# dpbriggs/Distributed-Sieve-e

Measured on AMD Instinct MI355X. Metric: sieved integers/sec at N=1e11, 1/2/4/8 MI355X; % of LDS/HBM roofline, higher is better.
Workload: dtype u32; 1 GPU; N=1e+11 odd-only chunked sieve, P=1 spread-work chunks (one per GPU), mask resident in HBM; N=100000000000, P=1, cs=49999999999, mask_bytes_per_gpu=6250000000, parallelism=range-partition x1 (RCCL broadcast + all-reduce)

## Files before the change

### distributed-sieve-e_amd/csrc/dse_host.cpp

```cpp
#include <rccl/rccl.h>

#include <algorithm>
#include <cmath>
#include <cstdio>
#include <cstring>
#include <string>
#include <vector>

#include "../../include/dse.h"
#include "dse_internal.h"

namespace {

thread_local std::string g_err;
thread_local int32_t g_code = DSE_OK;

int32_t fail(int32_t code, const std::string& msg) {
  g_err = msg;
  g_code = code;
  return code;
}

#define HIP_TRY(expr)                                                                     \
  do {                                                                                    \
    hipError_t e_ = (expr);                                                               \
    if (e_ != hipSuccess)                                                                 \
      return fail(DSE_EHIP, std::string(#expr " failed: ") + hipGetErrorString(e_));      \
  } while (0)

#define NCCL_TRY(expr)                                                                    \
  do {                                                                                    \
    ncclResult_t r_ = (expr);                                                             \
    if (r_ != ncclSuccess)                                                                \
      return fail(DSE_ENCCL, std::string(#expr " failed: ") + ncclGetErrorString(r_));    \
  } while (0)

uint64_t isqrt_u64(uint64_t x) {
  uint64_t r = (uint64_t)std::sqrt((long double)x);
  while (r > 0 && r * r > x) --r;
  while ((r + 1) * (r + 1) <= x) ++r;
  return r;
}

uint32_t prime_cap(uint64_t x) {
  if (x < 100) return 64;
  double b = 1.25506 * (double)x / std::log((double)x);
  return (uint32_t)b + 64;
}

struct ChunkMask {
  int32_t my_num = 0;
  uint64_t* dev_ptr = nullptr;
  uint64_t words = 0;
};

struct DevState {
  int device = 0;
  int num_cus = 0;
  hipStream_t stream = nullptr;
  void* table = nullptr;
  uint64_t table_bytes = 0;
  unsigned long long* counts = nullptr;
// ... 623 lines not shown
      return fail(DSE_EINVAL, "rccl_single needs a one-device context (dse_init(1) or dse_init_device)");
    if (value == 1 && ctx->comms.empty()) {
      int dev = ctx->devs[0].device;
      HIP_TRY(hipSetDevice(dev));
      ncclComm_t c;
      NCCL_TRY(ncclCommInitAll(&c, 1, &dev));
      ctx->comms.push_back(c);
    } else if (value == 0 && !ctx->comms.empty()) {
      HIP_TRY(hipSetDevice(ctx->devs[0].device));
      HIP_TRY(hipStreamSynchronize(ctx->devs[0].stream));
      NCCL_TRY(ncclCommDestroy(ctx->comms[0]));
      ctx->comms.clear();
    }
    ctx->rccl_single = value == 1;
    return DSE_OK;
  }
  if (n == "table_broadcast_max_bytes") {
    if (value < 0) return fail(DSE_EINVAL, "table_broadcast_max_bytes must be >= 0");
    ctx->opts.table_bcast_max = (uint64_t)value;
    return DSE_OK;
  }
  if (n == "bucket_cap_divisor") {
    if (value < 0 || value > 0xFFFFFFFFll) return fail(DSE_EINVAL, "bucket_cap_divisor out of range");
    ctx->opts.bucket_cap_div = (uint32_t)value;
    return DSE_OK;
  }
  return fail(DSE_EINVAL, "unknown option " + n);
}

int32_t dse_debug_get_stat(dse_ctx* ctx, const char* name, int64_t* value) {
  if (!ctx || !name || !value) return fail(DSE_EINVAL, "null ctx, stat name or value");
  const std::string n(name);
  if (n == "rccl_calls") {
    *value = ctx->rccl_calls;
    return DSE_OK;
  }
  if (n == "table_local_builds") {
    *value = ctx->table_local_builds;
    return DSE_OK;
  }
  if (n == "rccl_comms") {
    *value = (int64_t)ctx->comms.size();
    return DSE_OK;
  }
  if (n == "rccl_ranks") {
    int c = 0;
    if (!ctx->comms.empty()) NCCL_TRY(ncclCommCount(ctx->comms[0], &c));
    *value = c;
    return DSE_OK;
  }
  return fail(DSE_EINVAL, "unknown stat " + n);
}

}

namespace {

inline int fmt_u64(uint64_t v, char* out) {
  char t[24];
  int n = 0;
  do {
    t[n++] = (char)('0' + v % 10);
    v /= 10;
  } while (v);
  for (int i = 0; i < n; ++i) out[i] = t[n - 1 - i];
  return n;
}

inline int fmt_java_double(uint64_t v, char* out) {
  if (v < 10000000ull) {
    int n = fmt_u64(v, out);
    out[n++] = '.';
    out[n++] = '0';
    return n;
  }
  char d[24];
  int len = fmt_u64(v, d);
  int sig = len;
  while (sig > 1 && d[sig - 1] == '0') --sig;
  int n = 0;
  out[n++] = d[0];
  out[n++] = '.';
  if (sig == 1) out[n++] = '0';
  for (int i = 1; i < sig; ++i) out[n++] = d[i];
  out[n++] = 'E';
  n += fmt_u64((uint64_t)(len - 1), out + n);
  return n;
}

}

extern "C" int32_t dse_write_range_file(const char* path, int32_t my_num, uint64_t g_start, uint64_t nbits,
                                        const uint64_t* mask) {
  if (!path || !mask) return fail(DSE_EINVAL, "null path or mask");
  if (my_num < 1) return fail(DSE_EINVAL, "my_num must be >= 1");
  if (my_num == 1 && nbits < 4) return fail(DSE_EINVAL, "finish's 2/3/5/7 hack needs a chunk of >= 4 candidates");
  const uint64_t cs = nbits;
  FILE* f = std::fopen(path, "wb");
  if (!f) return fail(DSE_EIO, std::string("cannot open ") + path);
  std::vector<char> buf(1 << 20);
  size_t used = 0;
  int per_line = 0;
  const uint64_t base = g_start;
  auto emit = [&](uint64_t v) {
    if (used + 64 > buf.size()) {
      std::fwrite(buf.data(), 1, used, f);
// ... 47 lines not shown
```

### distributed-sieve-e_amd/csrc/dse_wheel_args.h

```cpp
#pragma once
#include <algorithm>
#include <vector>

#include "dse_wheel_geometry.h"

namespace dse {
namespace {

WheelRange make_wheel_range(const RangeSpec& rs, uint64_t* plane_lut) {
  WheelRange w{};
  const uint64_t v_start = 3 + 2 * rs.g_start;
  w.V0 = v_start - 1;
  w.nbits = rs.nbits;
  w.KB0 = w.V0 / 30;
  w.out = rs.out;
  w.count = rs.count;
  const uint32_t v0m = (uint32_t)(w.V0 % 30);
  uint32_t n = 0;
  *plane_lut = 0;
  for (uint32_t rho = 1; rho < 30; rho += 2) {
    const uint32_t r = (v0m + rho) % 30;
    if (r % 3 == 0 || r % 5 == 0) continue;
    uint32_t iota = 0;
    while (kR30[iota] != r) ++iota;
    w.rho_pack |= (uint64_t)rho << (5 * n);
    w.pl_pack |= n << (3 * iota);
    if (v0m + rho >= 30) w.e_iota |= 1u << iota;
    *plane_lut |= (uint64_t)n << (3 * (rho >> 1));
    ++n;
  }
  constexpr uint32_t small[] = {3, 5, 7, 11, 13, 17, 19, 23, 29, 31, 37, 41, 43, 47, 53, 59, 61, 67, 71, 73, 79};
  static_assert(small[sizeof(small) / sizeof(small[0]) - 1] == kQMax && (kQMax - 3) / 2 < 64, "fix covers 3..kQMax");
  for (uint32_t v : small)
    if (v >= v_start && (v - v_start) / 2 < rs.nbits) w.fix |= 1ull << ((v - v_start) / 2);
  for (int g = 0; g < kNG; ++g) w.v0g[g] = (uint16_t)(w.V0 % gmod(g));
  return w;
}

uint64_t isqrt64(uint64_t x) {
  uint64_t r = (uint64_t)__builtin_sqrt((double)x);
  while (r * r > x) --r;
  while ((r + 1) * (r + 1) <= x) ++r;
  return r;
}

WheelArgs make_wheel_args(const RangeSpec* rs, uint32_t n, uint64_t* plane_lut,
                          uint64_t wheel_max = kWheelMaxPrime) {
  static const std::vector<uint32_t> odd_primes = [] {
    std::vector<uint8_t> comp(kWheelMaxPrime / 2 + 1, 0);
    for (uint64_t i = 1; (2 * i + 1) * (2 * i + 1) <= kWheelMaxPrime; ++i)
      if (!comp[i])
        for (uint64_t j = ((2 * i + 1) * (2 * i + 1)) / 2; j <= kWheelMaxPrime / 2; j += 2 * i + 1) comp[j] = 1;
    std::vector<uint32_t> v;
    for (uint64_t i = 1; 2 * i + 1 <= kWheelMaxPrime; ++i)
      if (!comp[i]) v.push_back((uint32_t)(2 * i + 1));
    return v;
  }();
  const uint64_t lim[5] = {kQMax, TA, TB1, TB, std::min<uint64_t>(wheel_max, kWheelMaxPrime)};
  WheelArgs wa{};
  for (int t = 0; t < 5; ++t)
    wa.nthr[t] = (uint32_t)(std::upper_bound(odd_primes.begin(), odd_primes.end(), lim[t]) - odd_primes.begin());
  uint64_t seg = 0, lut = 0;
  for (uint32_t i = 0; i < n; ++i) {
    WheelRange& r = wa.r[i];
    r = make_wheel_range(rs[i], i ? &lut : plane_lut);
    r.seg0 = (uint32_t)seg;
    const uint64_t nseg_r = (rs[i].nbits + kWheelOutBits - 1) / kWheelOutBits;
    seg += nseg_r;
    r.lsh = 0;
    while (nseg_r > 0 && ((nseg_r - 1) >> r.lsh) >= kLPieces) ++r.lsh;
// ... 28 lines not shown
```

### distributed-sieve-e_amd/csrc/dse_wheel_geometry.h

```cpp
#pragma once
#include <hip/hip_runtime.h>
#include <stddef.h>
#include <stdint.h>

#include <algorithm>

#include "dse_internal.h"

namespace dse {
namespace {

constexpr uint32_t KP = 1u << kWheelLogKP;
constexpr uint32_t BLOCKS = KP / 32;
constexpr uint32_t IMG_WORDS = 8 * BLOCKS;
constexpr uint32_t IMG_BYTES = 4 * IMG_WORDS;
static_assert(IMG_BYTES == KP, "a period index is its block's byte address");
#define DSE_IMG_OFF_S "32768"
constexpr uint32_t kImgOff = 32768;
#define DSE_STR2(x) #x
#define DSE_STR(x) DSE_STR2(x)
constexpr uint32_t NT = 1024;
constexpr uint32_t NW = NT / 64;
static_assert(BLOCKS % (64 * NW) == 0, "expansion blocks");
#ifndef DSE_TA
// ... 26 lines not shown
constexpr uint32_t gmod(int g) { return kGQ[g][0] * kGQ[g][1] * kGQ[g][2]; }
constexpr uint32_t kInitWords = IMG_WORDS / NT;
constexpr uint32_t kInitRun = 32 * kInitWords;
constexpr uint32_t kExpandBlocks = BLOCKS / NW;
constexpr uint32_t kInitBlocks = kInitRun / 128 + 2;
constexpr uint32_t gdw(int g) { return ((gmod(g) + 32 * (4 * kInitBlocks + 1) + 127) / 128) * 4; }
constexpr uint32_t gbase(int g) { return g == 0 ? 0u : gbase(g - 1) + gdw(g - 1); }
constexpr uint32_t kGDW = gbase(kNG);
constexpr uint32_t kGInv30[kNG] = {inv30_const(gmod(0)), inv30_const(gmod(1)), inv30_const(gmod(2)),
                                   inv30_const(gmod(3)), inv30_const(gmod(4)), inv30_const(gmod(5)),
                                   inv30_const(gmod(6)), inv30_const(gmod(7)), inv30_const(gmod(8))};

struct InitTables {
  uint32_t w[4 * kGDW];
};
constexpr InitTables make_init_tables() {
  InitTables t{};
  for (int g = 0; g < kNG; ++g) {
    for (uint32_t j = 0; j < gdw(g) + 3; ++j) {
      uint32_t v = 0;
      for (uint32_t b = 0; b < 32; ++b) {
        const uint32_t y = 32 * j + b;
        const bool hit = y % kGQ[g][0] == 0 || y % kGQ[g][1] == 0 || (kGQ[g][2] > 1 && y % kGQ[g][2] == 0);
        v |= (uint32_t)hit << b;
      }
      for (uint32_t k = 0; k < 4; ++k)
        if (j >= k && j - k < gdw(g)) t.w[k * kGDW + gbase(g) + (j - k)] = v;
    }
  }
  return t;
}
__device__ const InitTables g_init_tables = make_init_tables();

constexpr uint32_t kLPieces = 16;
constexpr uint32_t kMaxRanges = 9;

}


struct WheelRange {
  uint64_t V0;
  uint64_t nbits;
  uint64_t KB0;
  uint64_t rho_pack;
  uint32_t* out;
  unsigned long long* count;
  uint32_t pl_pack;
  uint32_t e_iota;
  uint64_t fix;
  uint32_t seg0;
  uint16_t v0g[kNG];
  uint32_t lsh;
  uint32_t lcap[kLPieces];
};

struct WheelArgs {
  WheelRange r[kMaxRanges];
  uint32_t nranges;
  uint32_t nseg;
  uint32_t nthr[5];
  const uint32_t* bk_entries;
  const uint32_t* bk_start;
  const uint32_t* bk_reg0;
  const uint32_t* bk_n0;
  const unsigned long long* bk_spill;
  const uint32_t* bk_nspill;
  uint64_t bk_spill_cap;
  uint32_t bk_k0;
};
static_assert(sizeof(WheelArgs) <= 4096, "kernel arguments");
static_assert(alignof(WheelArgs) <= 8, "kernel argument layout");

namespace {

constexpr uint32_t kWaOffset = 8;

#ifndef DSE_BK_GRID
#define DSE_BK_GRID 1024
#endif
#ifndef DSE_BK_UNIT_BATCHES
#define DSE_BK_UNIT_BATCHES 4
#endif
constexpr uint32_t kBkBatchU = 16;
constexpr uint32_t kBkUnit = 64 * kBkBatchU * DSE_BK_UNIT_BATCHES;
constexpr uint32_t kBkGrid0 = DSE_BK_GRID;
#ifndef DSE_BK0_LISTS
#define DSE_BK0_LISTS 16
#endif
constexpr uint32_t kBk0Lists = DSE_BK0_LISTS;
static_assert(kBkGrid0 % kBk0Lists == 0 && 64 % kBk0Lists == 0, "band-0 bucket units");
constexpr uint32_t kKeyShift = 20;
static_assert(IMG_WORDS * 32 <= (1u << kKeyShift), "bucket entry layout");

}
}
```

### distributed-sieve-e_amd/csrc/dse_wheel_kernel.h

```cpp
#pragma once
#include "dse_wheel_geometry.h"

namespace dse {
namespace {

__device__ __forceinline__ uint32_t lds_addr(const uint32_t* p) {
  return (uint32_t)(uintptr_t)(const __attribute__((address_space(3))) uint32_t*)p;
}

__device__ __forceinline__ void lds_drain() { asm volatile("s_waitcnt lgkmcnt(0)" ::: "memory"); }

__device__ __forceinline__ uint32_t opaque(uint32_t x) {
  asm volatile("" : "+v"(x));
  return x;
}

constexpr uint32_t kBlockMask = ~31u;
#ifndef DSE_FAKE_CF_L
#define DSE_FAKE_CF_L 0
#endif
constexpr uint32_t kBlockMaskL = DSE_FAKE_CF_L ? ~127u : kBlockMask;
#ifndef DSE_FAKE_CF_INIT
#define DSE_FAKE_CF_INIT 0
#endif
#ifndef DSE_SHORT_TAIL
#define DSE_SHORT_TAIL 16
#endif
constexpr uint32_t kShortTail = DSE_SHORT_TAIL;
constexpr uint32_t odd_primes_upto(uint32_t x) {
  uint32_t c = 0;
  for (uint32_t v = 3; v <= x; v += 2) {
    bool pr = true;
    for (uint32_t d = 3; d * d <= v; d += 2)
      if (v % d == 0) { pr = false; break; }
    c += pr;
  }
  return c;
}
constexpr uint32_t kL0 = odd_primes_upto(TB);
constexpr uint32_t kLPrimeMask = 0x800FFFFFu;
static_assert(kWheelMaxPrime <= (1u << 20), "pl[] words: the L primes (odd, <= kWheelMaxPrime) are below 2^20");
__host__ __device__ constexpr uint32_t l_plan(uint32_t pmin, uint32_t pmax, uint32_t kp) {
  if (pmin > kp) return 2;
  if (pmin > kp / 2) return 1;
  const uint32_t n_min = pmax >= kp ? 0u : kp / pmax;
  const uint32_t n_all = (kp + pmin - 1) / pmin;
  return n_all - n_min <= kShortTail ? n_all << 3 : 4u | n_min << 3;
}
static_assert(l_plan(TB + 2, TB + 2, 1u << 17) < (1u << 11) && l_plan(TB + 2, TB + 2, 1u << 16) < (1u << 11),
              "the plan fits bits 20..30 of a pl[] word (bit 31: kLPrimeMask's dead-lane flag)");
static_assert(odd_primes_upto(kQMax) + kMidCap >= kL0, "the L list starts at kL0 whenever it exists");

__device__ __forceinline__ void mark_k(uint32_t pb4, uint32_t k, uint32_t one) {
// ... 126 lines not shown
  return (uint32_t)r;
}

__device__ __forceinline__ float fast_rcp(float x) { return __builtin_amdgcn_rcpf(x); }

__device__ __forceinline__ uint32_t div_ceil_small(uint32_t t, uint32_t p, float invp) {
  uint32_t q = (uint32_t)((float)t * invp);
  q = q * p > t ? q - 1 : q;
  q = (q + 1) * p <= t ? q + 1 : q;
  return q + (q * p != t ? 1u : 0u);
}

__device__ __forceinline__ uint32_t div_small(uint32_t t, uint32_t p, float invp) {
  uint32_t q = (uint32_t)((float)t * invp);
  q = q * p > t ? q - 1 : q;
  q = (q + 1) * p <= t ? q + 1 : q;
  return q;
}

__device__ __forceinline__ uint32_t mulmod_small(uint32_t x, uint32_t y, uint32_t p, float invp) {
  const uint32_t xy = x * y;
  uint32_t q = (uint32_t)((float)xy * invp);
  int32_t r = (int32_t)(xy - q * p);
  r = r < 0 ? r + (int32_t)p : r;
  r = r < 0 ? r + (int32_t)p : r;
  r = r >= (int32_t)p ? r - (int32_t)p : r;
  r = r >= (int32_t)p ? r - (int32_t)p : r;
  return (uint32_t)r;
}

__host__ __device__ __forceinline__ uint64_t inv30_of(uint64_t p) {
  constexpr uint64_t T = (14ull << 0) | (8ull << 12) | (9ull << 20) | (11ull << 24) | (3ull << 32) | (5ull << 36) |
                         (6ull << 44) | (0ull << 56);
  const uint32_t r = (uint32_t)(p % 30u);
  const uint64_t a = 2 * ((T >> (4 * (r >> 1))) & 15) + 1;
  return (p * a + 1) / 30;
}

__device__ __forceinline__ uint32_t plane_first(uint32_t Xs, uint32_t rho, uint32_t p, uint32_t inv30,
                                                float invp) {
  uint32_t t = Xs + rho;
  t = t >= p ? t - p : t;
  const uint32_t u = t ? p - t : 0u;
  return mulmod_small(u, inv30, p, invp);
}

__device__ __forceinline__ uint32_t first_at_or_after(uint32_t kp, uint32_t start, uint32_t p, float invp) {
  if (start <= kp) return kp;
  return kp + p * div_ceil_small(start - kp, p, invp);
}

__device__ __forceinline__ uint32_t kmin_for(uint32_t D, uint32_t rho) {
  return D > rho ? (D - rho + 29u) / 30u : 0u;
}

__device__ __forceinline__ uint32_t bfi(uint32_t m, uint32_t x, uint32_t y) {
  uint32_t r;
  asm("v_bfi_b32 %0, %1, %2, %3" : "=v"(r) : "s"(m), "v"(x), "v"(y));
  return r;
}

template <int S>
__device__ __forceinline__ void bit_block_swap(uint32_t& a, uint32_t& b) {
  constexpr uint32_t m = S == 4 ? 0x0F0F0F0Fu : S == 2 ? 0x33333333u : 0x55555555u;
  const uint32_t x = a, y = b;
  b = bfi(m, x >> S, y);
  a = bfi(~m, y << S, x);
}
__device__ __forceinline__ void bit_block_swaps(uint32_t (&W)[8]) {
  bit_block_swap<4>(W[0], W[4]); bit_block_swap<4>(W[1], W[5]);
  bit_block_swap<4>(W[2], W[6]); bit_block_swap<4>(W[3], W[7]);
  bit_block_swap<2>(W[0], W[2]); bit_block_swap<2>(W[1], W[3]);
  bit_block_swap<2>(W[4], W[6]); bit_block_swap<2>(W[5], W[7]);
  bit_block_swap<1>(W[0], W[1]); bit_block_swap<1>(W[2], W[3]);
  bit_block_swap<1>(W[4], W[5]); bit_block_swap<1>(W[6], W[7]);
}


template <int K>
__device__ __forceinline__ void a_classes(uint32_t pb4, uint32_t k, uint32_t p, uint32_t one) {
  const uint32_t D = p << 8;
#pragma unroll 1
  for (uint32_t r = 0; r < 32; ++r) {
    uint32_t a, bit;
    asm volatile(
        "v_and_or_b32 %0, %2, %3, %4\n\t"
        "v_lshlrev_b32 %1, %2, %5"
        : "=&v"(a), "=&v"(bit)
        : "v"(k), "s"(kBlockMask), "v"(pb4), "v"(one));
#pragma unroll
    for (int t = 0; t < K; ++t) {
      mark_at(a, bit);
      a += D;
    }
    mark_at(a, bit);
    k = opaque(k + p);
  }
}

struct MidRes {
  uint32_t* x;
  const uint32_t* inc;
  bool have;
};
__device__ __forceinline__ uint32_t mid_residue(const MidRes& mr, uint32_t i, uint32_t p, uint64_t m, uint64_t Vs,
                                                bool writer) {
  const uint32_t xs = mr.have ? mr.x[i] : mod_barrett(Vs, p, m);
  if (writer) {
    const uint32_t t = xs + mr.inc[i];
    mr.x[i] = min(t, t - p);
  }
  return xs;
}

__device__ __forceinline__ void unit_A(uint32_t img0, uint32_t pi, uint64_t m, const MidRes& mr, uint32_t idx,
                                       uint64_t Vs, uint64_t rho_pack, uint32_t lane, uint32_t one) {
  const uint32_t p = pi & 0xFFFFu, inv30 = pi >> 16;
  const uint64_t p2 = (uint64_t)p * p;
  const uint32_t Xs = __builtin_amdgcn_readfirstlane(mid_residue(mr, idx, p, m, Vs, lane == 0));
  const float invp = fast_rcp((float)p);
  const uint32_t pl = lane & 7, c = lane >> 3;
  const uint32_t rho = (uint32_t)(rho_pack >> (5 * pl)) & 31u;
  const uint32_t kp = plane_first(Xs, rho, p, inv30, invp);
  const uint32_t pb4 = img0 + 4 * pl;
  const uint32_t k = kp + 32 * c * p;
  if (p2 <= Vs) {
    switch (KP / (256 * p)) {
      case 1: a_classes<1>(pb4, k, p, one); return;
// ... 243 lines not shown
  } else {
    kbm = mod_barrett(Kb, p, o.m);
  }
  const uint32_t nKbm = 0u - kbm;
  const uint32_t pmax = __builtin_amdgcn_readlane(p, 63);
  const bool none = pmax > sqrt_vs;
  if (!none) {
    const uint32_t plan = (uint32_t)__builtin_amdgcn_readfirstlane(o.p) >> 20;
    const uint32_t n_run = plan >> 3;
    if ((plan & 3) == 2) unit_L_fast<2>(o, p, nKbm, ps, 0);
    else if ((plan & 3) == 1) unit_L_fast<1>(o, p, nKbm, ps, 0);
    else if (!(plan & 4)) unit_L_fast<0>(o, p, nKbm, ps, n_run);
    else unit_L_fast<0, true>(o, p, nKbm, ps, n_run);
    return;
  }
  const uint32_t pmin = __builtin_amdgcn_readfirstlane(p);
  const uint64_t p2 = (uint64_t)p * p;
  const bool live = p2 < Vend;
  const bool slow = p2 > Vs;
  const uint32_t D = slow && live ? (uint32_t)(p2 - Vs) : 0u;
  if (!live) return;
  const uint64_t rho_pack = *(volatile const uint64_t*)rho_pack_p;
#pragma unroll
  for (uint32_t q = 0; q < 8; ++q) {
    uint32_t kk = plane_start(o.a[q], nKbm, ps.ne[q], p);
    if (slow) {
      const uint32_t pl = (pl_rot >> (3 * q)) & 7u;
      const uint32_t rho = (uint32_t)(rho_pack >> (5 * pl)) & 31u;
      const uint32_t kmin = kmin_for(D, rho);
      if (kmin > kk) {
        const uint32_t d = kmin - kk;
        uint32_t qd = (uint32_t)((float)d * invp);
        while (qd * p < d) ++qd;
        while (qd > 0 && (qd - 1) * p >= d) --qd;
        kk += qd * p;
      }
    }
    const uint32_t pb4 = ps.pb[q];
    if (pmin > KP / 2) {
      mark_k(pb4, kk, ps.one);
      mark_k(pb4, kk + p, ps.one);
    } else {
      for (; kk < KP; kk += p) mark_k(pb4, kk, ps.one);
    }
  }
}

struct WheelLdsLow {
  uint64_t mid_m[kMidCap];
  uint32_t mid_p[kMidCap];
  uint32_t mid_x[kMidCap];
  uint32_t mid_inc[kMidCap];
  uint32_t x_seg;
  uint32_t lut[kMaxRanges][256];
  uint4 itab[kGDW];
  uint32_t thr[5];
  uint32_t ctr;
  unsigned long long rcnt[kMaxRanges];
};
static_assert(sizeof(WheelLdsLow) <= kImgOff, "LDS below the image");
struct WheelLds : WheelLdsLow {
  uint8_t pad[kImgOff - sizeof(WheelLdsLow)];
  uint32_t img[IMG_WORDS];
};
static_assert(sizeof(WheelLds) == kImgOff + IMG_BYTES, "the image ends the allocation");

template <bool BK>
__global__ __launch_bounds__(NT) void wheel_segments_kernel(const void* __restrict__ table, WheelArgs wa) {
  __shared__ WheelLds lds;
  uint64_t* const s_mid_m = lds.mid_m;
  uint32_t* const s_mid_p = lds.mid_p;
  uint32_t* const s_thr = lds.thr;

  const TableHeader* th = reinterpret_cast<const TableHeader*>(table);
  const uint32_t np = th->count;
  const uint32_t* __restrict__ P = reinterpret_cast<const uint32_t*>(reinterpret_cast<const char*>(table) + 16);
  const uint64_t* __restrict__ M =
      reinterpret_cast<const uint64_t*>(reinterpret_cast<const char*>(table) + table_m_offset(th->cap));
  const uint32_t* __restrict__ A =
      reinterpret_cast<const uint32_t*>(reinterpret_cast<const char*>(table) + table_a_offset(th->cap));
  const uint32_t* __restrict__ PL = reinterpret_cast<const uint32_t*>(reinterpret_cast<const char*>(table) +
                                                                    table_l_offset(th->cap)) +
                                    (kWheelLogKP == 17 ? 0u : th->cap);

#if defined(DSE_PAD_NOPS) && DSE_PAD_NOPS > 0
  asm volatile(".rept " DSE_STR(DSE_PAD_NOPS) "\n\ts_nop 0\n\t.endr");
#endif
  const uint32_t tid = threadIdx.x, lane_id = tid & 63, wave = tid >> 6;

  if (tid == 0) {
    s_thr[0] = min(wa.nthr[0], np);
    s_thr[1] = min(wa.nthr[1], np);
    s_thr[2] = min(wa.nthr[2], np);
    s_thr[3] = min(min(wa.nthr[3], np), s_thr[0] + kMidCap);
    s_thr[2] = min(s_thr[2], s_thr[3]);
    s_thr[4] = max(s_thr[3], min(wa.nthr[4], np));
    lds.ctr = 0;
    lds.x_seg = ~0u;
  }
  if (tid < kMaxRanges) lds.rcnt[tid] = 0;
  for (uint32_t x = tid; x < 256 * wa.nranges; x += NT) {
    const uint32_t v8 = x & 255;
    const uint64_t rho_pack = wa.r[x >> 8].rho_pack;
    uint32_t v = 0;
#pragma unroll
    for (uint32_t i = 0; i < 8; ++i) {
      const uint32_t rho = (uint32_t)(rho_pack >> (5 * i)) & 31u;
      if (!(v8 & (1u << i))) v |= 1u << ((rho - 1) >> 1);
    }
    lds.lut[x >> 8][v8 ^ (3u * (v8 >> 5))] = v;
  }
  for (uint32_t idx = tid; idx < 4 * kGDW; idx += NT) reinterpret_cast<uint32_t*>(lds.itab)[idx] = g_init_tables.w[idx];
  __syncthreads();
  const uint32_t i_mid0 = s_thr[0], i_midB = s_thr[1], i_midB2 = s_thr[2], i_mid1 = s_thr[3];
  for (uint32_t i = tid; i < i_mid1 - i_mid0; i += NT) {
    const uint32_t q = P[i_mid0 + i];
    s_mid_p[i] = q | ((uint32_t)inv30_of(q) << 16);
    s_mid_m[i] = M[i_mid0 + i];
    lds.mid_inc[i] = (uint32_t)(((uint64_t)gridDim.x * kWheelSpan) % q);
  }
  const uint32_t nA = i_midB - i_mid0;
  const uint32_t n_mid = i_mid1 - i_mid0;
  const uint32_t n_b1 = i_midB2 - i_mid0;
  const uint32_t nB1 = (i_midB2 - i_midB + 1) / 2;
  const uint32_t nB2 = (i_mid1 - i_midB2 + 7) / 8;
  const uint32_t i_big = s_thr[4];
  constexpr uint32_t kLU = 128;
  const uint32_t n1 = nA + nB1 + nB2;

  const uint32_t nseg = wa.nseg;
  const uint32_t grid = gridDim.x;
  const uint32_t T = blockIdx.x < nseg ? (nseg - 1 - blockIdx.x) / grid + 1 : 0u;
  auto range_of = [&](uint32_t g) -> uint32_t {
    uint32_t r = 0;
    for (uint32_t i = 1; i < wa.nranges; ++i) r = g >= wa.r[i].seg0 ? i : r;
    return r;
  };

  auto init_segment = [&](uint32_t* __restrict__ img, uint32_t g_seg) {
    const WheelRange& rg = wa.r[range_of(g_seg)];
    const uint64_t s = g_seg - rg.seg0;
    uint32_t lane = lane_id;
    asm volatile("" : "+v"(lane));
    const uint32_t pl = lane & 7, q = 8 * wave + (lane >> 3);
    const uint32_t rho = (uint32_t)(rg.rho_pack >> (5 * pl)) & 31u;
    constexpr uint32_t R = kInitWords;
    static_assert(R % 4 == 0, "staggered init runs");
    const uint32_t j = q & 3;
    const uint32_t b0 = 4 * R * (q >> 2) + (R + 1) * j;
    const uint32_t k0 = 32 * b0;
    constexpr uint32_t H = 16;
    static_assert(R % H == 0 && H % 4 == 0, "init passes");
    uint32_t boff[kNG], bsh[kNG];
    const uint32_t rho_o = opaque(rho), k0_o = opaque(k0);
#pragma unroll
    for (int g = 0; g < kNG; ++g) {
      const uint32_t Mg = gmod(g);
      const uint32_t wg = (uint32_t)(kWheelSpan % Mg);
      const uint32_t sg = (uint32_t)(s % Mg);
      const uint32_t x = ((uint32_t)rg.v0g[g] + sg * wg + rho_o) % Mg;
      const uint32_t o = (k0_o + x * kGInv30[g]) % Mg;
      const uint32_t d0 = o >> 5, kc = d0 & 3;
      boff[g] = (kc * kGDW + gbase(g) + d0 - kc) / 4;
#if DSE_FAKE_CF_INIT
      boff[g] = gbase(g) / 4 + (lane & 15u);
#endif
      bsh[g] = o & 31;
    }
    uint32_t* const wp = img + 8 * b0 + pl;
#pragma unroll
    for (uint32_t h = 0; h < R; h += H) {
      uint32_t acc[H];
#pragma unroll
      for (uint32_t r = 0; r < H; ++r) acc[r] = 0;
#pragma unroll
      for (int g = 0; g < kNG; ++g) {
        const uint4* bp = lds.itab + boff[g] + h / 4;
        uint32_t blk[H + 4];
#pragma unroll
        for (uint32_t b = 0; b < H / 4 + 1; ++b) {
          const uint4 v = bp[b];
          blk[4 * b] = v.x; blk[4 * b + 1] = v.y; blk[4 * b + 2] = v.z; blk[4 * b + 3] = v.w;
        }
#pragma unroll
        for (uint32_t r = 0; r < H; ++r) acc[r] |= __builtin_amdgcn_alignbit(blk[r + 1], blk[r], bsh[g]);
        asm volatile("" ::: "memory");
      }
#pragma unroll
      for (uint32_t r = 0; r < H; ++r) {
        if (h + r >= R - 3 && j == 3) continue;
        wp[8 * (h + r)] = acc[r];
      }
    }
    if (j != 3) {
      uint32_t acc = 0;
#pragma unroll
      for (int g = 0; g < kNG; ++g) {
        const uint4* bp = lds.itab + boff[g] + R / 4;
        const uint4 v = bp[0];
        acc |= __builtin_amdgcn_alignbit(v.y, v.x, bsh[g]);
      }
      wp[8 * R] = acc;
    }
  };

  auto expand_segment = [&](const uint32_t* __restrict__ img, uint32_t g_seg) {
    const uint32_t ri = range_of(g_seg);
    const WheelRange& rg = wa.r[ri];
    const uint64_t s = g_seg - rg.seg0;
    const uint64_t out_words = 2ull * ((rg.nbits + 63) / 64);
    uint32_t* __restrict__ out = rg.out;
    const uint32_t* __restrict__ s_lut = lds.lut[ri];
    uint32_t my_count = 0;
    uint32_t lane = lane_id;
    asm volatile("" : "+v"(lane));
    const uint32_t l = lane & 31;
    const uint32_t gsub = (l >= 4 && l < 12) || (l >= 16 && l < 20) || l >= 28;
    const uint32_t m = l < 4 ? l : l < 12 ? l - 4 : l < 20 ? l - 8 : l < 28 ? l - 12 : l - 16;
    const uint32_t bl = 16 * (2 * (lane >> 5) + gsub) + m;
    const uint64_t seg_word0 = s * (uint64_t)kOutWordsPerSeg;
#pragma unroll 1
    for (uint32_t t = 0; t < kExpandBlocks / 64; ++t) {
      const uint32_t blk = kExpandBlocks * wave + 64 * t + bl;
      const uint4* rp = reinterpret_cast<const uint4*>(img + 8 * blk);
      const uint4 lo = rp[0], hi = rp[1];
      uint32_t W[8] = {lo.x, lo.y, lo.z, lo.w, hi.x, hi.y, hi.z, hi.w};
      uint32_t n_comp = 0;
#pragma unroll
      for (int j = 0; j < 8; ++j) n_comp += __popc(W[j]);
      bit_block_swaps(W);
#pragma unroll
      for (int j = 0; j < 8; ++j) {
        const uint32_t h = (W[j] >> 5) & 0x07070707u;
        W[j] ^= h + (h << 1);
      }
      uint32_t o[15];
#pragma unroll
      for (int w = 0; w < 15; ++w) o[w] = 0;
#pragma unroll
      for (int q = 0; q < 4; ++q) {
#pragma unroll
        for (int j = 0; j < 8; ++j) {
          const uint32_t e = s_lut[(W[j] >> (8 * q)) & 0xFFu];
          const int pos = 15 * (8 * q + j);
          o[pos >> 5] |= e << (pos & 31);
          if ((pos & 31) > 17) o[(pos >> 5) + 1] |= e >> (32 - (pos & 31));
        }
      }
      const uint64_t w0 = seg_word0 + 15ull * blk;
      if (s == 0 && blk == 0) {
        o[0] |= (uint32_t)rg.fix;
        o[1] |= (uint32_t)(rg.fix >> 32);
      }
      const uint64_t bit0 = 32ull * w0;
      if (bit0 + 480 <= rg.nbits) {
        uint32_t cnt = 0;
        if (s == 0 && blk == 0) {
#pragma unroll
          for (int w = 0; w < 15; ++w) cnt += __popc(o[w]);
        } else {
          cnt = 256u - n_comp;
        }
        my_count += cnt;
        if (out) {
#pragma unroll
          for (int w = 0; w < 15; ++w) out[w0 + w] = o[w];
        }
      } else {
        const uint32_t rem = bit0 >= rg.nbits ? 0u : (uint32_t)(rg.nbits - bit0);
        uint32_t cnt = 0;
#pragma unroll
        for (int w = 0; w < 15; ++w) {
          const uint32_t b = 32u * w;
          o[w] = b >= rem ? 0u : (rem - b >= 32 ? o[w] : o[w] & ((1u << (rem - b)) - 1u));
          cnt += __popc(o[w]);
        }
        my_count += cnt;
        if (out) {
#pragma unroll
          for (int w = 0; w < 15; ++w)
            if (w0 + w < out_words) out[w0 + w] = o[w];
        }
      }
    }
#pragma unroll
    for (int o = 32; o > 0; o >>= 1) my_count += __shfl_xor(my_count, o);
    if (lane == 0 && my_count) atomicAdd(&lds.rcnt[ri], (unsigned long long)my_count);
  };

  auto mark_segment = [&](uint32_t* __restrict__ img, uint32_t g_seg) {
    const WheelRange& rg = wa.r[range_of(g_seg)];
    const uint64_t s = g_seg - rg.seg0;
    const uint64_t Vs = rg.V0 + s * kWheelSpan;
    const uint64_t Vend = Vs + kWheelSpan;
    uint32_t lane = lane_id;
    asm volatile("" : "+v"(lane));
    const uint32_t img0 = lds_addr(img) - kImgOff;
    const uint32_t one = opaque(1u);
    uint32_t bk_b0 = 0, bk_b1 = 0, n0u = 0, n1u = 0, n3 = 0;
    if (BK) {
      n0u = wa.bk_k0 ? kBkGrid0 / kBk0Lists : 0u;
      bk_b0 = wa.bk_start[s];
      bk_b1 = wa.bk_start[s + 1];
      n1u = (bk_b1 - bk_b0 + kBkUnit - 1) / kBkUnit;
      n3 = n0u + n1u + (wa.bk_k0 && *wa.bk_nspill ? 1u : 0u);
    }
    const uint64_t* rho_pack_p = reinterpret_cast<const uint64_t*>(
        (const char*)__builtin_amdgcn_kernarg_segment_ptr() + kWaOffset +
        range_of(g_seg) * sizeof(WheelRange) + offsetof(WheelRange, rho_pack));
    uint32_t sqrt_vs = (uint32_t)__builtin_sqrt((double)Vs);
    while ((uint64_t)sqrt_vs * sqrt_vs > Vs) --sqrt_vs;
    while ((uint64_t)(sqrt_vs + 1) * (sqrt_vs + 1) <= Vs) ++sqrt_vs;
    sqrt_vs = __builtin_amdgcn_readfirstlane(sqrt_vs);
    uint32_t sqrt_ve = (uint32_t)__builtin_sqrt((double)(Vend - 1));
    while ((uint64_t)sqrt_ve * sqrt_ve > Vend - 1) --sqrt_ve;
    while ((uint64_t)(sqrt_ve + 1) * (sqrt_ve + 1) <= Vend - 1) ++sqrt_ve;
    sqrt_ve = __builtin_amdgcn_readfirstlane(sqrt_ve);
    const uint32_t rot = (i_mid1 + lane) & 7;
    const uint32_t pl_rot = ((rg.pl_pack >> (3 * rot)) | (rg.pl_pack << (24 - 3 * rot))) & 0xFFFFFFu;
    const uint32_t e_rot = ((rg.e_iota >> rot) | (rg.e_iota << (8 - rot))) & 0xFFu;
    PlaneSteps ps;
    ps.one = one;
#pragma unroll
    for (uint32_t q = 0; q < 8; ++q) {
      ps.pb[q] = img0 + 4 * ((pl_rot >> (3 * q)) & 7u) + (DSE_FAKE_CF_L ? ((lane_id >> 3) & 3u) << 5 : 0u);
      ps.ne[q] = 0u - ((e_rot >> q) & 1u);
    }
    const uint64_t Kb = rg.KB0 + s * (uint64_t)KP;
    const bool need_m = BK && Kb >= (1ull << 38);
    MidRes mr;
    mr.x = lds.mid_x;
    mr.inc = lds.mid_inc;
    mr.have = __builtin_amdgcn_readfirstlane(lds.x_seg) == g_seg;
    const uint32_t i_live = max(i_mid1, min(i_big, rg.lcap[min((uint32_t)(s >> rg.lsh), kLPieces - 1)]));
    const uint32_t n2 = (i_live - i_mid1 + kLU - 1) / kLU;
    const uint32_t n_int = min(n1, n2), n_all = n1 + n2;
    const uint32_t ctr_addr = lds_addr(&lds.ctr);
    auto claim = [&]() -> uint32_t {
      uint32_t j = 0;
      if (lane == 0) asm volatile("ds_add_rtn_u32 %0, %1, %2" : "=v"(j) : "v"(ctr_addr), "v"(1u) : "memory");
// ... 156 lines not shown
```

### distributed-sieve-e_amd/mail_sieve_e/_dse.py

```python
from __future__ import annotations

import ctypes
import os

_HERE = os.path.dirname(os.path.abspath(__file__))
LIB_PATH = os.path.join(_HERE, "libdse.so")
CSRC = os.path.normpath(os.path.join(_HERE, "..", "csrc"))

DSE_OK = 0
ERRORS = {
    -1: "DSE_EINVAL",
    -2: "DSE_EHIP",
    -3: "DSE_ENCCL",
    -4: "DSE_ENOMEM",
    -5: "DSE_EIO",
    -6: "DSE_ERANGE",
    -7: "DSE_EINTERNAL",
}

_i32, _i64, _u64 = ctypes.c_int32, ctypes.c_int64, ctypes.c_uint64
_vp, _cp = ctypes.c_void_p, ctypes.c_char_p
_pi64, _pu64 = ctypes.POINTER(_i64), ctypes.POINTER(_u64)
SIGNATURES = {
    "dse_version": (_cp, []),
    "dse_last_error": (_cp, []),
    "dse_last_status": (_i32, []),
    "dse_device_count": (_i32, []),
    "dse_init": (_vp, [_i32]),
    "dse_init_device": (_vp, [_i32]),
    "dse_destroy": (None, [_vp]),
    "dse_ctx_num_devices": (_i32, [_vp]),
    "dse_spread_work": (_i32, [_i64, _i32, _pi64, _pi64]),
    "dse_tail_range": (_i32, [_i64, _i32, _pu64, _pu64]),
    "dse_sieve_chunk": (_i32, [_vp, _i64, _i32, _i32, _pu64, _pu64]),
    "dse_sieve_odd_range": (_i32, [_vp, _u64, _u64, _pu64, _pu64]),
    "dse_sieve_all": (_i32, [_vp, _i64, _i32, _pu64, _pu64, _pu64]),
    "dse_copy_chunk_mask": (_i32, [_vp, _i32, _pu64]),
    "dse_sieve_window": (_i32, [_vp, _u64, _u64, _pu64]),
    "dse_write_primes_file": (_i32, [_cp, _i32, _i64, _i32, _pu64]),
    "dse_write_range_file": (_i32, [_cp, _i32, _u64, _u64, _pu64]),
    "dse_base_table_bytes": (_u64, [_u64]),
    "dse_base_limit_max": (_u64, []),
    "dse_base_limit_for_range": (_u64, [_u64, _u64]),
    "dse_base_primes_dev_async": (_i32, [_vp, _u64, _vp, _u64, _vp]),
    "dse_base_table_prime_bytes": (_u64, [_u64]),
    "dse_base_table_broadcast_bytes": (_u64, [_u64]),
    "dse_base_table_finish_dev_async": (_i32, [_vp, _u64, _vp, _u64, _vp]),
    "dse_sieve_range_dev_async": (_i32, [_vp, _vp, _u64, _u64, _vp, _vp, _vp]),
    "dse_device_status": (_i32, [_vp]),
    "dse_debug_set_option": (_i32, [_vp, _cp, _i64]),
    "dse_debug_init_logical": (_vp, [_i32]),
    "dse_debug_get_stat": (_i32, [_vp, _cp, _pi64]),
}

_lib = None


class DseError(RuntimeError):
    def __init__(self, code: int, where: str, msg: str):
        super().__init__(f"{where}: {ERRORS.get(code, code)}: {msg}")
        self.code = code


def lib() -> ctypes.CDLL:
    global _lib
    if _lib is None:
        if not os.path.exists(LIB_PATH):
            raise ImportError(
                f"libdse.so not built at {LIB_PATH}; run `make -C {CSRC}` "
                "(the HIP extension is required, there is no CPU fallback)")
        try:
            import torch
        except ImportError:
            pass
        L = ctypes.CDLL(LIB_PATH)
        for name, (res, args) in SIGNATURES.items():
            if name.startswith("dse_debug_") and not hasattr(L, name):
                continue
            f = getattr(L, name)
            f.restype = res
            f.argtypes = args
        _lib = L
    return _lib


def check(rc: int, where: str) -> None:
    if rc != DSE_OK:
        raise DseError(rc, where, lib().dse_last_error().decode(errors="replace"))


def u64p(arr):
    if arr is None:
        return None
    return arr.ctypes.data_as(_pu64)
```

### include/dse.h

```cpp
#ifndef DSE_H
#define DSE_H

#include <stdint.h>

#ifdef __cplusplus
extern "C" {
#endif

#define DSE_OK 0
#define DSE_EINVAL -1
#define DSE_EHIP -2
#define DSE_ENCCL -3
#define DSE_ENOMEM -4
#define DSE_EIO -5
#define DSE_ERANGE -6
#define DSE_EINTERNAL -7

typedef struct dse_ctx dse_ctx;

const char *dse_version(void);

const char *dse_last_error(void);

int32_t dse_last_status(void);
// ... 12 lines not shown

int32_t dse_tail_range(int64_t n, int32_t P, uint64_t *g_start, uint64_t *nbits);

int32_t dse_sieve_chunk(dse_ctx *ctx, int64_t n, int32_t P, int32_t my_num,
                        uint64_t *mask_or_null, uint64_t *count);

int32_t dse_sieve_odd_range(dse_ctx *ctx, uint64_t g_start, uint64_t nbits,
                            uint64_t *mask_or_null, uint64_t *count);

int32_t dse_sieve_all(dse_ctx *ctx, int64_t n, int32_t P, uint64_t *per_chunk_counts,
                      uint64_t *pi_ref, uint64_t *pi_full);

int32_t dse_copy_chunk_mask(dse_ctx *ctx, int32_t my_num, uint64_t *mask);

int32_t dse_sieve_window(dse_ctx *ctx, uint64_t lo, uint64_t hi, uint64_t *count);

int32_t dse_write_primes_file(const char *path, int32_t my_num, int64_t n, int32_t P,
                              const uint64_t *mask);

int32_t dse_write_range_file(const char *path, int32_t my_num, uint64_t g_start, uint64_t nbits,
                             const uint64_t *mask);


uint64_t dse_base_table_bytes(uint64_t limit);

uint64_t dse_base_limit_max(void);

uint64_t dse_base_limit_for_range(uint64_t g_start, uint64_t nbits);

int32_t dse_base_primes_dev_async(dse_ctx *ctx, uint64_t limit, void *table_dev,
                                  uint64_t table_bytes, void *stream);

uint64_t dse_base_table_prime_bytes(uint64_t limit);

#define DSE_TABLE_BROADCAST_MAX_BYTES (8ull << 20)
uint64_t dse_base_table_broadcast_bytes(uint64_t limit);

int32_t dse_base_table_finish_dev_async(dse_ctx *ctx, uint64_t limit, void *table_dev,
                                        uint64_t table_bytes, void *stream);

int32_t dse_sieve_range_dev_async(dse_ctx *ctx, const void *table_dev, uint64_t g_start,
                                  uint64_t nbits, uint64_t *mask_dev, uint64_t *count_dev,
                                  void *stream);

int32_t dse_device_status(dse_ctx *ctx);


int32_t dse_debug_set_option(dse_ctx *ctx, const char *name, int64_t value);

int32_t dse_debug_get_stat(dse_ctx *ctx, const char *name, int64_t *value);

dse_ctx *dse_debug_init_logical(int32_t num_logical);

#ifdef __cplusplus
}
#endif

#endif
```

Before: 17740 billion integers/s.

## Replace LDS lookup-table bit expansion with compile-time specialized bit-matrix transpose

Changes how each 8-plane wheel-30 block is expanded into 15 odd-only output words. The old path did a partial bit-block swap followed by per-byte lookups into a per-range LDS table. The new path runs a full 16-row butterfly transpose using v_bfi, templated on the range's residue variant (V0 mod 30)/2, so zero rows are pruned at compile time, and dispatches on that variant with a wave-uniform switch. This drops the LDS lookup table, its setup loop and the LDS reads, which also frees shared memory. The cost is more ALU work per block, 15 instantiated code copies that enlarge the kernel, and possibly more register pressure. A host debug entry point is added for testing the expansion.

```diff
diff --git a/distributed-sieve-e_amd/csrc/dse_expand_bits.h b/distributed-sieve-e_amd/csrc/dse_expand_bits.h
--- /dev/null
+++ b/distributed-sieve-e_amd/csrc/dse_expand_bits.h
@@ -0,0 +1,133 @@
+#pragma once
+#include <hip/hip_runtime.h>
+#include <stdint.h>
+
+#include "dse_internal.h"
+
+namespace dse {
+
+constexpr int kExpandVariants = 15;
+
+struct ExpandPlan {
+  uint8_t slot[8];
+  uint16_t nz[5];
+};
+
+constexpr ExpandPlan make_expand_plan(int T) {
+  ExpandPlan p{};
+  bool used[15] = {};
+  for (int j = 0; j < 8; ++j) used[((int)(kR30[j] - 1) / 2 + 15 - T) % 15] = true;
+  int n = 0;
+  uint32_t nz = 0;
+  for (int s = 0; s < 15; ++s)
+    if (used[s]) {
+      p.slot[n++] = (uint8_t)s;
+      nz |= 1u << s;
+    }
+  p.nz[0] = (uint16_t)nz;
+  for (int st = 0; st < 4; ++st) {
+    const int S = 8 >> st;
+    uint32_t next = 0;
+    for (int r = 0; r < 16; ++r)
+      if (!(r & S) && ((nz >> r | nz >> (r + S)) & 1u)) next |= 1u << r | 1u << (r + S);
+    nz = next;
+    p.nz[st + 1] = (uint16_t)nz;
+  }
+  return p;
+}
+
+struct ExpandMasks {
+  uint32_t m8, m4, m2, m1;
+};
+__host__ __device__ __forceinline__ ExpandMasks expand_masks() {
+  ExpandMasks k{0x00FF00FFu, 0x0F0F0F0Fu, 0x33333333u, 0x55555555u};
+#if defined(__HIP_DEVICE_COMPILE__)
+  asm volatile("" : "+s"(k.m8), "+s"(k.m4), "+s"(k.m2), "+s"(k.m1));
+#endif
+  return k;
+}
+
+template <int S, bool NZA, bool NZB>
+__host__ __device__ __forceinline__ void expand_row_swap(uint32_t& a, uint32_t& b, const ExpandMasks& k) {
+  constexpr uint32_t m = S == 8 ? 0x00FF00FFu : S == 4 ? 0x0F0F0F0Fu : S == 2 ? 0x33333333u : 0x55555555u;
+  const uint32_t x = a, y = b;
+  if (NZA && NZB) {
+#if defined(__HIP_DEVICE_COMPILE__)
+    const uint32_t ms = S == 8 ? k.m8 : S == 4 ? k.m4 : S == 2 ? k.m2 : k.m1;
+    asm("v_bfi_b32 %0, %1, %2, %3" : "=v"(b) : "s"(ms), "v"(x >> S), "v"(y));
+    asm("v_bfi_b32 %0, %1, %2, %3" : "=v"(a) : "s"(ms), "v"(x), "v"(y << S));
+#else
+    (void)k;
+    b = ((x >> S) & m) | (y & ~m);
+    a = ((y << S) & ~m) | (x & m);
+#endif
+  } else if (NZA) {
+    a = x & m;
+    b = (x >> S) & m;
+  } else if (NZB) {
+    a = (y << S) & ~m;
+    b = y & ~m;
+  }
+}
+
+template <int T, int ST, int R>
+__host__ __device__ __forceinline__ void expand_stage_row(uint32_t (&Z)[16], const ExpandMasks& k) {
+  constexpr ExpandPlan plan = make_expand_plan(T);
+  constexpr int S = 8 >> ST;
+  if constexpr (!(R & S))
+    expand_row_swap<S, (plan.nz[ST] >> R & 1) != 0, (plan.nz[ST] >> (R + S) & 1) != 0>(Z[R], Z[R + S], k);
+  if constexpr (R + 1 < 16) expand_stage_row<T, ST, R + 1>(Z, k);
+}
+
+template <int T>
+__host__ __device__ __forceinline__ void expand_block(const uint32_t (&P)[8], uint32_t (&o)[15],
+                                                      const ExpandMasks& k) {
+  static_assert(T >= 0 && T < kExpandVariants, "variant = (V0 mod 30) / 2");
+  constexpr ExpandPlan plan = make_expand_plan(T);
+  uint32_t Z[16];
+#pragma unroll
+  for (int r = 0; r < 16; ++r) Z[r] = 0;
+#pragma unroll
+  for (int i = 0; i < 8; ++i) Z[plan.slot[i]] = ~P[i];
+  expand_stage_row<T, 0, 0>(Z, k);
+  expand_stage_row<T, 1, 0>(Z, k);
+  expand_stage_row<T, 2, 0>(Z, k);
+  expand_stage_row<T, 3, 0>(Z, k);
+#pragma unroll
+  for (int w = 0; w < 15; ++w) o[w] = 0;
+#pragma unroll
+  for (int c = 0; c < 16; ++c) {
+    const int rot = (15 * c) & 31;
+    const uint32_t r = rot ? (Z[c] << rot) | (Z[c] >> (32 - rot)) : Z[c];
+#pragma unroll
+    for (int h = 0; h < 2; ++h) {
+      const int pos = 15 * (c + 16 * h), w = pos >> 5, p = pos & 31;
+      o[w] |= r & (0x7FFFu << p);
+      if (p > 17) o[w + 1] |= r & ((1u << (p - 17)) - 1u);
+    }
+  }
+}
+
+inline bool expand_block_variant(int variant, const uint32_t (&P)[8], uint32_t (&o)[15]) {
+  const ExpandMasks k = expand_masks();
+  switch (variant) {
+    case 0: expand_block<0>(P, o, k); return true;
+    case 1: expand_block<1>(P, o, k); return true;
+    case 2: expand_block<2>(P, o, k); return true;
+    case 3: expand_block<3>(P, o, k); return true;
+    case 4: expand_block<4>(P, o, k); return true;
+    case 5: expand_block<5>(P, o, k); return true;
+    case 6: expand_block<6>(P, o, k); return true;
+    case 7: expand_block<7>(P, o, k); return true;
+    case 8: expand_block<8>(P, o, k); return true;
+    case 9: expand_block<9>(P, o, k); return true;
+    case 10: expand_block<10>(P, o, k); return true;
+    case 11: expand_block<11>(P, o, k); return true;
+    case 12: expand_block<12>(P, o, k); return true;
+    case 13: expand_block<13>(P, o, k); return true;
+    case 14: expand_block<14>(P, o, k); return true;
+    default: return false;
+  }
+}
+
+}
diff --git a/distributed-sieve-e_amd/csrc/dse_host.cpp b/distributed-sieve-e_amd/csrc/dse_host.cpp
--- a/distributed-sieve-e_amd/csrc/dse_host.cpp
+++ b/distributed-sieve-e_amd/csrc/dse_host.cpp
@@ -8,6 +8,7 @@
 #include <vector>
 
 #include "../../include/dse.h"
+#include "dse_expand_bits.h"
 #include "dse_internal.h"
 
 namespace {
@@ -737,6 +738,15 @@
   return fail(DSE_EINVAL, "unknown stat " + n);
 }
 
+int32_t dse_debug_expand_block(int32_t variant, const uint32_t planes[8], uint32_t out[15]) {
+  if (!planes || !out) return fail(DSE_EINVAL, "null planes or out");
+  uint32_t p[8], o[15];
+  std::memcpy(p, planes, sizeof p);
+  if (!dse::expand_block_variant(variant, p, o)) return fail(DSE_EINVAL, "expand variant outside 0..14");
+  std::memcpy(out, o, sizeof o);
+  return DSE_OK;
+}
+
 }
 
 namespace {
diff --git a/distributed-sieve-e_amd/csrc/dse_wheel_args.h b/distributed-sieve-e_amd/csrc/dse_wheel_args.h
--- a/distributed-sieve-e_amd/csrc/dse_wheel_args.h
+++ b/distributed-sieve-e_amd/csrc/dse_wheel_args.h
@@ -16,6 +16,7 @@
   w.out = rs.out;
   w.count = rs.count;
   const uint32_t v0m = (uint32_t)(w.V0 % 30);
+  w.variant = v0m / 2;
   uint32_t n = 0;
   *plane_lut = 0;
   for (uint32_t rho = 1; rho < 30; rho += 2) {
diff --git a/distributed-sieve-e_amd/csrc/dse_wheel_geometry.h b/distributed-sieve-e_amd/csrc/dse_wheel_geometry.h
--- a/distributed-sieve-e_amd/csrc/dse_wheel_geometry.h
+++ b/distributed-sieve-e_amd/csrc/dse_wheel_geometry.h
@@ -102,6 +102,7 @@
   uint16_t v0g[kNG];
   uint32_t lsh;
   uint32_t lcap[kLPieces];
+  uint32_t variant;
 };
 
 struct WheelArgs {
diff --git a/distributed-sieve-e_amd/csrc/dse_wheel_kernel.h b/distributed-sieve-e_amd/csrc/dse_wheel_kernel.h
--- a/distributed-sieve-e_amd/csrc/dse_wheel_kernel.h
+++ b/distributed-sieve-e_amd/csrc/dse_wheel_kernel.h
@@ -1,4 +1,7 @@
 #pragma once
+#include <type_traits>
+
+#include "dse_expand_bits.h"
 #include "dse_wheel_geometry.h"
 
 namespace dse {
@@ -231,28 +234,6 @@
 
 __device__ __forceinline__ uint32_t kmin_for(uint32_t D, uint32_t rho) {
   return D > rho ? (D - rho + 29u) / 30u : 0u;
-}
-
-__device__ __forceinline__ uint32_t bfi(uint32_t m, uint32_t x, uint32_t y) {
-  uint32_t r;
-  asm("v_bfi_b32 %0, %1, %2, %3" : "=v"(r) : "s"(m), "v"(x), "v"(y));
-  return r;
-}
-
-template <int S>
-__device__ __forceinline__ void bit_block_swap(uint32_t& a, uint32_t& b) {
-  constexpr uint32_t m = S == 4 ? 0x0F0F0F0Fu : S == 2 ? 0x33333333u : 0x55555555u;
-  const uint32_t x = a, y = b;
-  b = bfi(m, x >> S, y);
-  a = bfi(~m, y << S, x);
-}
-__device__ __forceinline__ void bit_block_swaps(uint32_t (&W)[8]) {
-  bit_block_swap<4>(W[0], W[4]); bit_block_swap<4>(W[1], W[5]);
-  bit_block_swap<4>(W[2], W[6]); bit_block_swap<4>(W[3], W[7]);
-  bit_block_swap<2>(W[0], W[2]); bit_block_swap<2>(W[1], W[3]);
-  bit_block_swap<2>(W[4], W[6]); bit_block_swap<2>(W[5], W[7]);
-  bit_block_swap<1>(W[0], W[1]); bit_block_swap<1>(W[2], W[3]);
-  bit_block_swap<1>(W[4], W[5]); bit_block_swap<1>(W[6], W[7]);
 }
 
 
@@ -602,7 +583,6 @@
   uint32_t mid_x[kMidCap];
   uint32_t mid_inc[kMidCap];
   uint32_t x_seg;
-  uint32_t lut[kMaxRanges][256];
   uint4 itab[kGDW];
   uint32_t thr[5];
   uint32_t ctr;
@@ -649,17 +629,6 @@
     lds.x_seg = ~0u;
   }
   if (tid < kMaxRanges) lds.rcnt[tid] = 0;
-  for (uint32_t x = tid; x < 256 * wa.nranges; x += NT) {
-    const uint32_t v8 = x & 255;
-    const uint64_t rho_pack = wa.r[x >> 8].rho_pack;
-    uint32_t v = 0;
-#pragma unroll
-    for (uint32_t i = 0; i < 8; ++i) {
-      const uint32_t rho = (uint32_t)(rho_pack >> (5 * i)) & 31u;
-      if (!(v8 & (1u << i))) v |= 1u << ((rho - 1) >> 1);
-    }
-    lds.lut[x >> 8][v8 ^ (3u * (v8 >> 5))] = v;
-  }
   for (uint32_t idx = tid; idx < 4 * kGDW; idx += NT) reinterpret_cast<uint32_t*>(lds.itab)[idx] = g_init_tables.w[idx];
   __syncthreads();
   const uint32_t i_mid0 = s_thr[0], i_midB = s_thr[1], i_midB2 = s_thr[2], i_mid1 = s_thr[3];
@@ -754,13 +723,12 @@
     }
   };
 
-  auto expand_segment = [&](const uint32_t* __restrict__ img, uint32_t g_seg) {
-    const uint32_t ri = range_of(g_seg);
+  auto expand_blocks = [&](const uint32_t* __restrict__ img, uint32_t g_seg, uint32_t ri, auto vt) {
+    constexpr int VT = decltype(vt)::value;
     const WheelRange& rg = wa.r[ri];
     const uint64_t s = g_seg - rg.seg0;
     const uint64_t out_words = 2ull * ((rg.nbits + 63) / 64);
     uint32_t* __restrict__ out = rg.out;
-    const uint32_t* __restrict__ s_lut = lds.lut[ri];
     uint32_t my_count = 0;
     uint32_t lane = lane_id;
     asm volatile("" : "+v"(lane));
@@ -769,6 +737,7 @@
     const uint32_t m = l < 4 ? l : l < 12 ? l - 4 : l < 20 ? l - 8 : l < 28 ? l - 12 : l - 16;
     const uint32_t bl = 16 * (2 * (lane >> 5) + gsub) + m;
     const uint64_t seg_word0 = s * (uint64_t)kOutWordsPerSeg;
+    const ExpandMasks masks = expand_masks();
 #pragma unroll 1
     for (uint32_t t = 0; t < kExpandBlocks / 64; ++t) {
       const uint32_t blk = kExpandBlocks * wave + 64 * t + bl;
@@ -778,25 +747,8 @@
       uint32_t n_comp = 0;
 #pragma unroll
       for (int j = 0; j < 8; ++j) n_comp += __popc(W[j]);
-      bit_block_swaps(W);
-#pragma unroll
-      for (int j = 0; j < 8; ++j) {
-        const uint32_t h = (W[j] >> 5) & 0x07070707u;
-        W[j] ^= h + (h << 1);
-      }
       uint32_t o[15];
-#pragma unroll
-      for (int w = 0; w < 15; ++w) o[w] = 0;
-#pragma unroll
-      for (int q = 0; q < 4; ++q) {
-#pragma unroll
-        for (int j = 0; j < 8; ++j) {
-          const uint32_t e = s_lut[(W[j] >> (8 * q)) & 0xFFu];
-          const int pos = 15 * (8 * q + j);
-          o[pos >> 5] |= e << (pos & 31);
-          if ((pos & 31) > 17) o[(pos >> 5) + 1] |= e >> (32 - (pos & 31));
-        }
-      }
+      expand_block<VT>(W, o, masks);
       const uint64_t w0 = seg_word0 + 15ull * blk;
       if (s == 0 && blk == 0) {
         o[0] |= (uint32_t)rg.fix;
@@ -836,6 +788,18 @@
 #pragma unroll
     for (int o = 32; o > 0; o >>= 1) my_count += __shfl_xor(my_count, o);
     if (lane == 0 && my_count) atomicAdd(&lds.rcnt[ri], (unsigned long long)my_count);
+  };
+  auto expand_segment = [&](const uint32_t* __restrict__ img, uint32_t g_seg) {
+    const uint32_t ri = range_of(g_seg);
+    switch (__builtin_amdgcn_readfirstlane(wa.r[ri].variant)) {
+#define DSE_EXPAND_CASE(V) \
+  case V: expand_blocks(img, g_seg, ri, std::integral_constant<int, V>{}); break;
+      DSE_EXPAND_CASE(0) DSE_EXPAND_CASE(1) DSE_EXPAND_CASE(2) DSE_EXPAND_CASE(3) DSE_EXPAND_CASE(4)
+      DSE_EXPAND_CASE(5) DSE_EXPAND_CASE(6) DSE_EXPAND_CASE(7) DSE_EXPAND_CASE(8) DSE_EXPAND_CASE(9)
+      DSE_EXPAND_CASE(10) DSE_EXPAND_CASE(11) DSE_EXPAND_CASE(12) DSE_EXPAND_CASE(13) DSE_EXPAND_CASE(14)
+#undef DSE_EXPAND_CASE
+      default: break;
+    }
   };
 
   auto mark_segment = [&](uint32_t* __restrict__ img, uint32_t g_seg) {
diff --git a/distributed-sieve-e_amd/mail_sieve_e/_dse.py b/distributed-sieve-e_amd/mail_sieve_e/_dse.py
--- a/distributed-sieve-e_amd/mail_sieve_e/_dse.py
+++ b/distributed-sieve-e_amd/mail_sieve_e/_dse.py
@@ -51,6 +51,7 @@
     "dse_debug_set_option": (_i32, [_vp, _cp, _i64]),
     "dse_debug_init_logical": (_vp, [_i32]),
     "dse_debug_get_stat": (_i32, [_vp, _cp, _pi64]),
+    "dse_debug_expand_block": (_i32, [_i32, ctypes.POINTER(ctypes.c_uint32), ctypes.POINTER(ctypes.c_uint32)]),
 }
 
 _lib = None
diff --git a/include/dse.h b/include/dse.h
--- a/include/dse.h
+++ b/include/dse.h
@@ -88,6 +88,8 @@
 
 dse_ctx *dse_debug_init_logical(int32_t num_logical);
 
+int32_t dse_debug_expand_block(int32_t variant, const uint32_t planes[8], uint32_t out[15]);
+
 #ifdef __cplusplus
 }
 #endif
```

Measured after the change: 18210 billion integers/s (median of 6 runs). 2.7% higher.
